# pedropro/UrsoNet

Measured on AMD Instinct MI355X. Metric: images/sec fwd+bwd ResNet50 640x512 bs32/GPU, higher is better.
Workload: dtype bf16; 1 GPU; resnet50 bottleneck=32 ori_resolution=16 soft-class head + loc regression, batch 32/GPU x 512x640x3, full training step (prep+fwd+loss+bwd+clip+SGD); global_batch=32, parallelism=dp1, comm_cus=0, hipgraph=True, runner=Engine, input=uint8 frames in HBM, mean subtraction + cast in the step (molding kernel), gradient_norm_from_finalisation_blocks=True, weight_gradients_on_forked_stream=True

## Files before the change

ursonet_amd/csrc/conv_c3.hip:

```cpp
#include "lds_mfma.h"
#include "internal.h"
#include <utility>

struct C3Args {
    const void* src; const void* wgt; const float* bias; const void* mask; void* dst;
    uint32_t bytes;
    int B, H, W, tiles_x, tiles_y, ntiles;
    int relu;
};

constexpr int C3_TH = 4, C3_TW = 32, C3_HW = C3_TW + 2, C3_HROWS = (C3_TH + 2) * C3_HW;
constexpr int C3_NA = 7;
constexpr int C3_ABUF = 224 * 128, C3_OOFF = 2 * C3_ABUF, C3_BOFF = C3_OOFF + C3_TH * C3_TW * 128, C3_LDS = C3_BOFF + 256;

__device__ __forceinline__ uint32_t c3_rd(int row, int h, int j) {
    const int s = (row >> 1) & 7;
    return (uint32_t)(row * 128 + ((((2 * j + h) ^ s)) << 4));
}

template <typename T, bool MASK>
__global__ __launch_bounds__(256, 2) void c3_kernel(const C3Args a) {
    static_assert(sizeof(T) == 2, "16-bit element types only");
    __shared__ __attribute__((aligned(1024))) char smem[C3_LDS];
    const uint32_t lds0 = (uint32_t)(uintptr_t)(__attribute__((address_space(3))) char*)smem;
    const int tid = threadIdx.x, lane = tid & 63, wave = __builtin_amdgcn_readfirstlane(tid >> 6);
    const int cw = wave & 1, pw = wave >> 1;
    int l31 = lane & 31;
    const int h = lane >> 5;

    const UrsoTileStream ts = urso_tile_stream(a.ntiles);
    const int t_end = ts.t_end, bpx = ts.bpx;
    int tile = ts.tile;
    if (tile >= t_end) return;

    const i32x4_t rs = raw_rsrc(a.src, a.bytes);
    const __amdgpu_buffer_rsrc_t rds = make_rsrc(a.dst, a.bytes);
    const __amdgpu_buffer_rsrc_t rmk = make_rsrc(MASK ? a.mask : a.dst, MASK ? a.bytes : 0u);

    int lane_d = lane;
    auto tile_origin = [&](int t, int& b, int& y0, int& x0) {
        const int tx = t % a.tiles_x, q = t / a.tiles_x;
        const int ty = q % a.tiles_y;
        b = q / a.tiles_y; y0 = ty * C3_TH; x0 = tx * C3_TW;
    };
    auto dma_tile = [&](int t, int buf) {
        int b, y0, x0;
        tile_origin(t, b, y0, x0);
        const int base = ((b * a.H + y0 - 1) * a.W + x0 - 1) * 128;
        asm volatile("" : "+v"(lane_d));
#pragma unroll
        for (int i = 0; i < C3_NA; ++i) {
            const int hr = 8 * (wave + 4 * i) + (lane_d >> 3);
            const int hy = (hr * 241) >> 13, hx = hr - hy * C3_HW;
            const int y = y0 - 1 + hy, x = x0 - 1 + hx;
            const bool ok = hr < C3_HROWS && y >= 0 && y < a.H && x >= 0 && x < a.W;
            const uint32_t off = (uint32_t)(base + (hy * a.W + hx) * 128 + (((lane_d & 7) ^ ((hx >> 1) & 7)) << 4));
            lds_dma16(rs, lds0 + buf * C3_ABUF + (wave + 4 * i) * 1024, ok ? off : URSO_OOB_SHIFT);
        }
    };

    i32x4_t wfr[9][4];
    {
        const int lg = 16 * ((l31 >> 2) & 1) + 4 * (l31 >> 3) + (l31 & 3);
        const char* wrow = (const char*)a.wgt + (size_t)(32 * cw + lg) * (9 * 64 * 2);
#pragma unroll
        for (int t = 0; t < 9; ++t)
#pragma unroll
            for (int j = 0; j < 4; ++j) wfr[t][j] = *(const i32x4_t*)(wrow + (t * 64 + 16 * j + 8 * h) * 2);
    }
    if (tid < 64) *(float*)(smem + C3_BOFF + tid * 4) = a.bias ? a.bias[tid] : 0.f;

    constexpr int NST = 4;
    uint32_t ea[3];
#pragma unroll
    for (int kx = 0; kx < 3; ++kx) ea[kx] = (uint32_t)(l31 * 128 + ((h ^ (((l31 + kx) >> 1) & 7)) << 4));

    dma_tile(tile, 0);
    int buf = 0;
    bool first = true;
    while (true) {
        const bool has_next = tile + bpx < t_end;
        if (first) wait_vm<0>(); else wait_vm<NST>();
        first = false;
        lds_barrier_asm();
        if (has_next) dma_tile(tile + bpx, buf ^ 1);

        f32x16_t acc[2];
        {
            const f32x4_t* bp = (const f32x4_t*)(smem + C3_BOFF + (32 * cw + 16 * h) * 4);
#pragma unroll
            for (int q = 0; q < 4; ++q) {
                const f32x4_t b4 = bp[q];
#pragma unroll
                for (int r = 0; r < 2; ++r) { acc[r][4 * q] = b4.x; acc[r][4 * q + 1] = b4.y; acc[r][4 * q + 2] = b4.z; acc[r][4 * q + 3] = b4.w; }
            }
        }
        i32x4_t f[4];
        uint32_t eb[3];
#pragma unroll
        for (int kx = 0; kx < 3; ++kx) eb[kx] = ea[kx] + (uint32_t)(buf * C3_ABUF + 2 * pw * C3_HW * 128);
        auto rd = [&](i32x4_t& fs, int s) {
            const int hr = s / 12, kx = (s / 4) % 3, j = s & 3;
            if (j == 0) asm volatile("" : "+v"(eb[kx]));
            fs = *(const i32x4_t*)(smem + (hr * C3_HW + kx) * 128 + (eb[kx] ^ (uint32_t)(j << 5)));
        };
        rd(f[0], 0);
        rd(f[1], 1);
        rd(f[2], 2);
#pragma unroll
        for (int s = 0; s < 48; ++s) {
            if (s + 3 < 48) rd(f[(s + 3) & 3], s + 3);
            __builtin_amdgcn_sched_barrier(0);
            const int hr = s / 12, kx = (s / 4) % 3, j = s & 3;
            if (hr <= 2) Mma32<T>::run(wfr[3 * hr + kx][j], f[s & 3], acc[0]);
            if (hr >= 1) Mma32<T>::run(wfr[3 * (hr - 1) + kx][j], f[s & 3], acc[1]);
            __builtin_amdgcn_sched_barrier(0);
        }

        char* sO = smem + C3_OOFF;
#pragma unroll
        for (int r = 0; r < 2; ++r) {
            const int px = (2 * pw + r) * 32 + l31;
#pragma unroll
            for (int v = 0; v < 2; ++v) {
                T o[8];
#pragma unroll
                for (int e = 0; e < 8; ++e) { float y = acc[r][8 * v + e]; y = a.relu ? relu_f(y) : y; o[e] = Elem<T>::from_f(y); }
                i32x4_t ov; __builtin_memcpy(&ov, o, 16);
                *(i32x4_t*)(sO + px * 128 + (((4 * cw + 2 * h + v) ^ ((px >> 1) & 7)) << 4)) = ov;
            }
        }
        int b, y0, x0;
        tile_origin(tile, b, y0, x0);
        uint32_t so[NST];
        i32x4_t mv[NST];
#pragma unroll
        for (int i = 0; i < NST; ++i) {
            const int row = 8 * (wave + 4 * i) + (lane >> 3);
            const int y = y0 + (row >> 5), x = x0 + (row & 31);
            so[i] = (y < a.H && x < a.W) ? (uint32_t)(((b * a.H + y) * a.W + x) * 128 + (((lane & 7) ^ ((row >> 1) & 7)) << 4)) : URSO_OOB_SHIFT;
            if constexpr (MASK) mv[i] = buf_load16(rmk, so[i]);
        }
        lds_barrier_asm();
#pragma unroll
        for (int i = 0; i < NST; ++i) {
            i32x4_t v = *(const i32x4_t*)(sO + (wave + 4 * i) * 1024 + lane * 16);
            if constexpr (MASK) {
                T x[8], m[8];
                __builtin_memcpy(x, &v, 16); __builtin_memcpy(m, &mv[i], 16);
#pragma unroll
                for (int e = 0; e < 8; ++e) x[e] = Elem<T>::to_f(m[e]) > 0.f ? x[e] : Elem<T>::from_f(0.f);
                __builtin_memcpy(&v, x, 16);
            }
            buf_store16(rds, so[i], v);
        }
        if (!has_next) break;
        tile += bpx; buf ^= 1;
    }
}

constexpr int C3W_PATCH = 2 * C3_ABUF;
constexpr int C3W_EOFF = 2 * C3W_PATCH, C3W_BOFF = C3W_EOFF + 8192, C3W_LDS = C3W_BOFF + 512;
constexpr int C3W_NA = 7;

template <typename T, bool MASK, int TW>
__global__ __launch_bounds__(512, 2) void c3w_kernel(const C3Args a) {
    constexpr int TH = 128 / TW, HW = TW + 2, HROWS = (TH + 2) * HW;
    static_assert(TW == 32 || TW == 16, "tile width");
    static_assert(sizeof(T) == 2, "16-bit element types only");
    __shared__ __attribute__((aligned(1024))) char smem[C3W_LDS];
    const uint32_t lds0 = (uint32_t)(uintptr_t)(__attribute__((address_space(3))) char*)smem;
    const int tid = threadIdx.x, lane = tid & 63, wave = __builtin_amdgcn_readfirstlane(tid >> 6);
    const int fq = wave & 3, ch = wave >> 2;
    int l31 = lane & 31;
    const int h = lane >> 5;

    const UrsoTileStream ts = urso_tile_stream(a.ntiles);
    const int t_end = ts.t_end, bpx = ts.bpx;
    int tile = ts.tile;
    if (tile >= t_end) return;

    const i32x4_t rs = raw_rsrc(a.src, a.bytes);
    const __amdgpu_buffer_rsrc_t rds = make_rsrc(a.dst, a.bytes);
    const __amdgpu_buffer_rsrc_t rmk = make_rsrc(MASK ? a.mask : a.dst, MASK ? a.bytes : 0u);

    int lane_d = lane;
    auto tile_origin = [&](int t, int& b, int& y0, int& x0) {
        const int tx = t % a.tiles_x, q = t / a.tiles_x;
        const int ty = q % a.tiles_y;
        b = q / a.tiles_y; y0 = ty * TH; x0 = tx * TW;
    };
    auto dma_tile = [&](int t, int buf) {
        int b, y0, x0;
        tile_origin(t, b, y0, x0);
        const int base = ((b * a.H + y0 - 1) * a.W + x0 - 1) * 256;
        asm volatile("" : "+v"(lane_d));
#pragma unroll
        for (int i = 0; i < C3W_NA; ++i) {
            const int ii = wave + 8 * i, half = ii >= 26 ? 1 : 0, rb = ii - 26 * half;
            const int hr = 8 * rb + (lane_d >> 3);
            const int hy = TW == 32 ? ((hr * 241) >> 13) : ((hr * 3641) >> 16), hx = hr - hy * HW;
            const int y = y0 - 1 + hy, x = x0 - 1 + hx;
            const bool ok = ii < 52 && hr < HROWS && y >= 0 && y < a.H && x >= 0 && x < a.W;
            const int sw = (hx >> 1) & 7;
            const uint32_t off = (uint32_t)(base + (hy * a.W + hx) * 256 + half * 128 + (((lane_d & 7) ^ sw) << 4));
            if (ii < 54) lds_dma16(rs, lds0 + buf * C3W_PATCH + half * C3_ABUF + rb * 1024, ok ? off : URSO_OOB_SHIFT);
        }
    };

    i32x4_t wfr[9][4];
    {
        const int lg = 16 * ((l31 >> 2) & 1) + 4 * (l31 >> 3) + (l31 & 3);
        const char* wrow = (const char*)a.wgt + (size_t)(32 * fq + lg) * (9 * 128 * 2);
#pragma unroll
        for (int t = 0; t < 9; ++t)
#pragma unroll
            for (int j = 0; j < 4; ++j) wfr[t][j] = *(const i32x4_t*)(wrow + (t * 128 + 64 * ch + 16 * j + 8 * h) * 2);
    }
    if (tid < 128) *(float*)(smem + C3W_BOFF + tid * 4) = a.bias ? a.bias[tid] : 0.f;

    constexpr int NST = 4;
    uint32_t ea[3];
    {
        const int prow = TW == 32 ? l31 : (l31 >> 4) * HW + (l31 & 15);
#pragma unroll
        for (int kx = 0; kx < 3; ++kx) ea[kx] = (uint32_t)(prow * 128 + ((h ^ ((((l31 & (TW - 1)) + kx) >> 1) & 7)) << 4));
    }
    dma_tile(tile, 0);
    int buf = 0;
    bool first = true;
    while (true) {
        const bool has_next = tile + bpx < t_end;
        if (first) wait_vm<0>(); else wait_vm<NST>();
        first = false;
        lds_barrier_asm();
        if (has_next) dma_tile(tile + bpx, buf ^ 1);
        f32x16_t acc[4];
#pragma unroll
        for (int r = 0; r < 4; ++r)
#pragma unroll
            for (int e = 0; e < 16; ++e) acc[r][e] = 0.f;
        i32x4_t f[4];
        uint32_t eb[3];
#pragma unroll
        for (int kx = 0; kx < 3; ++kx) eb[kx] = ea[kx] + (uint32_t)(buf * C3W_PATCH + ch * C3_ABUF);
        auto fresh = [&](int s) { if ((s & 3) == 0) asm volatile("" : "+v"(eb[(s / 4) % 3])); };
        if constexpr (TW == 32) {
            auto rd = [&](i32x4_t& fs, int s) {
                const int hr = s / 12, kx = (s / 4) % 3, j = s & 3;
                fresh(s);
                fs = *(const i32x4_t*)(smem + (hr * HW + kx) * 128 + (eb[kx] ^ (uint32_t)(j << 5)));
            };
            rd(f[0], 0);
            rd(f[1], 1);
            rd(f[2], 2);
#pragma unroll
            for (int s = 0; s < 72; ++s) {
                if (s + 3 < 72) rd(f[(s + 3) & 3], s + 3);
                __builtin_amdgcn_sched_barrier(0);
                const int hr = s / 12, kx = (s / 4) % 3, j = s & 3;
#pragma unroll
                for (int r = 0; r < 4; ++r) {
                    const int ky = hr - r;
                    if (ky >= 0 && ky <= 2) Mma32<T>::run(wfr[3 * ky + kx][j], f[s & 3], acc[r]);
                }
                __builtin_amdgcn_sched_barrier(0);
            }
        } else {
            auto rd = [&](i32x4_t& fs, int s) {
                const int rp = s / 12, kx = (s / 4) % 3, j = s & 3;
                fresh(s);
                fs = *(const i32x4_t*)(smem + (rp * HW + kx) * 128 + (eb[kx] ^ (uint32_t)(j << 5)));
            };
            rd(f[0], 0);
            rd(f[1], 1);
#pragma unroll
            for (int s = 0; s < 108; ++s) {
                if (s + 2 < 108) rd(f[(s + 2) % 3], s + 2);
                __builtin_amdgcn_sched_barrier(0);
                const int rp = s / 12, kx = (s / 4) % 3, j = s & 3;
#pragma unroll
                for (int m = 0; m < 4; ++m) {
                    const int ky = rp - 2 * m;
                    if (ky >= 0 && ky <= 2) Mma32<T>::run(wfr[3 * ky + kx][j], f[s % 3], acc[m]);
                }
                __builtin_amdgcn_sched_barrier(0);
            }
        }

        char* sX = smem + buf * C3W_PATCH;
        auto xoff = [&](int w, int rr, int q) -> char* {
            const uint32_t o = (uint32_t)(w * 8192 + ((rr * 4 + q) * 64 + lane) * 16);
            return (o < (uint32_t)C3W_PATCH) ? sX + o : smem + C3W_EOFF + (o - C3W_PATCH);
        };
        lds_barrier_asm();
#pragma unroll
        for (int rr = 0; rr < 2; ++rr) {
            const f32x16_t& v = (ch == 0) ? acc[2 + rr] : acc[rr];
#pragma unroll
            for (int q = 0; q < 4; ++q) *(f32x4_t*)xoff(wave, rr, q) = f32x4_t{v[4 * q], v[4 * q + 1], v[4 * q + 2], v[4 * q + 3]};
        }
        lds_barrier_asm();
        f32x16_t fin[2];
#pragma unroll
        for (int rr = 0; rr < 2; ++rr) {
            fin[rr] = (ch == 0) ? acc[rr] : acc[2 + rr];
#pragma unroll
            for (int q = 0; q < 4; ++q) {
                const f32x4_t p = *(const f32x4_t*)xoff(wave ^ 4, rr, q);
                fin[rr][4 * q] += p.x; fin[rr][4 * q + 1] += p.y; fin[rr][4 * q + 2] += p.z; fin[rr][4 * q + 3] += p.w;
            }
        }
        lds_barrier_asm();
        char* sO = sX;
        {
            const f32x4_t* bp = (const f32x4_t*)(smem + C3W_BOFF + (32 * fq + 16 * h) * 4);
#pragma unroll
            for (int rr = 0; rr < 2; ++rr) {
                const int px = (2 * ch + rr) * 32 + l31;
#pragma unroll
                for (int v = 0; v < 2; ++v) {
                    const f32x4_t b0 = bp[2 * v], b1 = bp[2 * v + 1];
                    const float bb[8] = {b0.x, b0.y, b0.z, b0.w, b1.x, b1.y, b1.z, b1.w};
                    T o[8];
#pragma unroll
                    for (int e = 0; e < 8; ++e) { float y = fin[rr][8 * v + e] + bb[e]; y = a.relu ? relu_f(y) : y; o[e] = Elem<T>::from_f(y); }
                    i32x4_t ov; __builtin_memcpy(&ov, o, 16);
                    *(i32x4_t*)(sO + px * 256 + (((4 * fq + 2 * h + v) ^ (px & 15)) << 4)) = ov;
                }
            }
        }
        int b, y0, x0;
        tile_origin(tile, b, y0, x0);
        uint32_t so[NST];
        i32x4_t mv[NST];
#pragma unroll
        for (int i = 0; i < NST; ++i) {
            const int p = (wave + 8 * i) * 64 + lane, px = p >> 4;
            const int y = y0 + px / TW, x = x0 + px % TW;
            so[i] = (y < a.H && x < a.W) ? (uint32_t)(((b * a.H + y) * a.W + x) * 256 + (((p & 15) ^ (px & 15)) << 4)) : URSO_OOB_SHIFT;
            if constexpr (MASK) mv[i] = buf_load16(rmk, so[i]);
        }
        lds_barrier_asm();
#pragma unroll
        for (int i = 0; i < NST; ++i) {
            i32x4_t v = *(const i32x4_t*)(sO + (wave + 8 * i) * 1024 + lane * 16);
            if constexpr (MASK) {
                T x[8], m[8];
                __builtin_memcpy(x, &v, 16); __builtin_memcpy(m, &mv[i], 16);
#pragma unroll
                for (int e = 0; e < 8; ++e) x[e] = Elem<T>::to_f(m[e]) > 0.f ? x[e] : Elem<T>::from_f(0.f);
                __builtin_memcpy(&v, x, 16);
            }
            buf_store16(rds, so[i], v);
        }
        if (!has_next) break;
        tile += bpx; buf ^= 1;
    }
}


#ifdef C3V_OLD_SWZ
__device__ __forceinline__ uint32_t c3v_swz(int col) { return (uint32_t)(col & 15); }
#else
__device__ __forceinline__ uint32_t c3v_swz(int col) { return (uint32_t)(0xfe64dcba98643210ull >> (4 * (col & 15))) & 15u; }
#endif
constexpr int C3V_HW = 18, C3V_HPIX = 10 * C3V_HW, C3V_PATCH = C3V_HPIX * 256;
constexpr int C3V_NA = 6;
#ifndef C3V_PF
#define C3V_PF 3
#endif
#ifndef C3V_DBG
#define C3V_DBG 0
#endif
#ifdef C3V_SEQ
__host__ __device__ constexpr int c3v_step(int t) { return t; }
#else
__host__ __device__ constexpr int c3v_step(int t) { return (t >> 1) + (t & 1) * 60; }
#endif
#ifdef C3V_NOSB
#define C3V_SB() do {} while (0)
#else
#define C3V_SB() __builtin_amdgcn_sched_barrier(0)
#endif
constexpr int C3V_OOFF = 2 * C3V_PATCH, C3V_BOFF = C3V_OOFF + 2 * 128 * 256, C3V_LDS = C3V_BOFF + 512;

template <class F, int... I> __device__ __forceinline__ void c3_static_for_impl(F&& f, std::integer_sequence<int, I...>) { (f(std::integral_constant<int, I>{}), ...); }
template <int N, class F> __device__ __forceinline__ void c3_static_for(F&& f) { c3_static_for_impl(static_cast<F&&>(f), std::make_integer_sequence<int, N>{}); }

template <typename T, bool MASK>
__global__ __launch_bounds__(512, 2) void c3v_kernel(const C3Args a) {
    static_assert(sizeof(T) == 2, "16-bit element types only");
    __shared__ __attribute__((aligned(1024))) char smem[C3V_LDS];
    const uint32_t lds0 = (uint32_t)(uintptr_t)(__attribute__((address_space(3))) char*)smem;
    const int tid = threadIdx.x, lane = tid & 63, wave = __builtin_amdgcn_readfirstlane(tid >> 6);
    const int fr = lane & 15, fg = lane >> 4;

    const UrsoTileStream ts = urso_tile_stream(a.ntiles);
    const int t_end = ts.t_end, bpx = ts.bpx;
    int tile = ts.tile;
    if (tile >= t_end) return;

    const i32x4_t rs = raw_rsrc(a.src, a.bytes);
    const __amdgpu_buffer_rsrc_t rds = make_rsrc(a.dst, a.bytes);
    const __amdgpu_buffer_rsrc_t rmk = make_rsrc(MASK ? a.mask : a.dst, MASK ? a.bytes : 0u);

    int lane_d = lane;
    auto tile_origin = [&](int t, int& b, int& y0, int& x0) {
        const int tx = t % a.tiles_x, q = t / a.tiles_x;
        const int ty = q % a.tiles_y;
        b = q / a.tiles_y; y0 = ty * 8; x0 = tx * 16;
    };
    auto dma_tile = [&](int t, int buf) {
        int b, y0, x0;
        tile_origin(t, b, y0, x0);
        const int base = ((b * a.H + y0 - 1) * a.W + x0 - 1) * 256;
        asm volatile("" : "+v"(lane_d));
#pragma unroll
        for (int i = 0; i < C3V_NA; ++i) {
            const int ii = wave + 8 * i;
            const int hp = 4 * ii + (lane_d >> 4);
            const int hy = (hp * 3641) >> 16, hx = hp - hy * C3V_HW;
            const int y = y0 - 1 + hy, x = x0 - 1 + hx;
            const bool ok = ii < 45 && y >= 0 && y < a.H && x >= 0 && x < a.W;
            const uint32_t off = (uint32_t)(base + (hy * a.W + hx) * 256 + (((uint32_t)(lane_d & 15) ^ c3v_swz(hx)) << 4));
            if (ii < 45) lds_dma16(rs, lds0 + buf * C3V_PATCH + ii * 1024, ok ? off : URSO_OOB_SHIFT);
        }
    };

    i32x4_t wfr[9][4];
    {
        const char* wrow = (const char*)a.wgt + (size_t)(16 * wave + fr) * (9 * 128 * 2);
#pragma unroll
        for (int t = 0; t < 9; ++t)
#pragma unroll
            for (int j = 0; j < 4; ++j) wfr[t][j] = *(const i32x4_t*)(wrow + (t * 128 + 32 * j + 8 * fg) * 2);
    }
    if (tid < 128) *(float*)(smem + C3V_BOFF + tid * 4) = a.bias ? a.bias[tid] : 0.f;

    uint32_t ea[3];
#pragma unroll
    for (int kx = 0; kx < 3; ++kx) ea[kx] = (uint32_t)((fr + kx) * 256) + (((uint32_t)fg ^ c3v_swz(fr + kx)) << 4);
    constexpr int NST = 4;
    uint32_t so[NST] = {URSO_OOB_SHIFT, URSO_OOB_SHIFT, URSO_OOB_SHIFT, URSO_OOB_SHIFT};
    i32x4_t mv[NST];
    auto flush = [&](int ob) {
        const char* sO = smem + C3V_OOFF + ob * (128 * 256);
#pragma unroll
        for (int i = 0; i < NST; ++i) {
            i32x4_t v = *(const i32x4_t*)(sO + (wave + 8 * i) * 1024 + lane * 16);
            if constexpr (MASK) {
                T x[8], m[8];
                __builtin_memcpy(x, &v, 16); __builtin_memcpy(m, &mv[i], 16);
#pragma unroll
                for (int e = 0; e < 8; ++e) x[e] = Elem<T>::to_f(m[e]) > 0.f ? x[e] : Elem<T>::from_f(0.f);
                __builtin_memcpy(&v, x, 16);
            }
            buf_store16(rds, so[i], v);
        }
    };
    dma_tile(tile, 0);
    int buf = 0, ob = 0;
    bool pend = false;
    while (true) {
        const bool has_next = tile + bpx < t_end;
        wait_vm<0>();
        lds_barrier_asm();
        if (has_next) dma_tile(tile + bpx, buf ^ 1);
        if (pend) flush(ob ^ 1);
        f32x4_t acc[8];
#pragma unroll
        for (int r = 0; r < 8; ++r) acc[r] = f32x4_t{0.f, 0.f, 0.f, 0.f};
        uint32_t eb[3];
#pragma unroll
        for (int kx = 0; kx < 3; ++kx) eb[kx] = ea[kx] + (uint32_t)(buf * C3V_PATCH);
        constexpr int PF = C3V_PF, RING = PF + 1;
        i32x4_t f[RING];
        auto rd = [&](i32x4_t& fs, int s) {
            const int hr = s / 12, kx = (s / 4) % 3, j = s & 3;
            if ((s & 3) == 0) asm volatile("" : "+v"(eb[kx]));
            if (!(C3V_DBG & 2) || s < PF) fs = *(const i32x4_t*)(smem + hr * C3V_HW * 256 + (eb[kx] ^ (uint32_t)(j << 6)));
        };
#pragma unroll
        for (int t = 0; t < PF; ++t) rd(f[t], c3v_step(t));
        c3_static_for<120>([&](auto sc) {
            constexpr int t = decltype(sc)::value, s = c3v_step(t);
            if constexpr (t + PF < 120) rd(f[(t + PF) % RING], c3v_step(t + PF));
            C3V_SB();
            constexpr int hr = s / 12, kx = (s / 4) % 3, j = s & 3;
            if (!(C3V_DBG & 1)) {
                if constexpr (hr >= 0 && hr < 8) Mma<T>::run(wfr[kx][j], f[t % RING], acc[hr]);
                if constexpr (hr - 1 >= 0 && hr - 1 < 8) Mma<T>::run(wfr[3 + kx][j], f[t % RING], acc[hr - 1]);
                if constexpr (hr - 2 >= 0 && hr - 2 < 8) Mma<T>::run(wfr[6 + kx][j], f[t % RING], acc[hr - 2]);
            }
            C3V_SB();
        });
        if (C3V_DBG & 4) { if (!has_next) break; tile += bpx; buf ^= 1; continue; }

        {
            char* sO = smem + C3V_OOFF + ob * (128 * 256);
            const f32x4_t bq = *(const f32x4_t*)(smem + C3V_BOFF + (16 * wave + 4 * fg) * 4);
#pragma unroll
            for (int r = 0; r < 8; ++r) {
                const int px = 16 * r + fr;
                float y0v = acc[r].x + bq.x, y1v = acc[r].y + bq.y, y2v = acc[r].z + bq.z, y3v = acc[r].w + bq.w;
                if (a.relu) { y0v = relu_f(y0v); y1v = relu_f(y1v); y2v = relu_f(y2v); y3v = relu_f(y3v); }
                T o[4] = {Elem<T>::from_f(y0v), Elem<T>::from_f(y1v), Elem<T>::from_f(y2v), Elem<T>::from_f(y3v)};
                i32x2_t ov; __builtin_memcpy(&ov, o, 8);
                *(i32x2_t*)(sO + px * 256 + ((((2 * wave + (fg >> 1)) ^ (px & 15))) << 4) + (fg & 1) * 8) = ov;
            }
        }
        {
            int b, y0, x0;
            tile_origin(tile, b, y0, x0);
#pragma unroll
            for (int i = 0; i < NST; ++i) {
                const int p = (wave + 8 * i) * 64 + lane, px = p >> 4;
                const int y = y0 + (px >> 4), x = x0 + (px & 15);
                so[i] = (y < a.H && x < a.W) ? (uint32_t)(((b * a.H + y) * a.W + x) * 256 + (((p & 15) ^ (px & 15)) << 4)) : URSO_OOB_SHIFT;
                if constexpr (MASK) mv[i] = buf_load16(rmk, so[i]);
            }
        }
        pend = true;
        if (!has_next) break;
        tile += bpx; buf ^= 1; ob ^= 1;
    }
    if constexpr (MASK) wait_vm<0>();
    lds_barrier_asm();
    flush(ob);
}

static int c3w_util(int H, int W, int tw) {
    const int th = 128 / tw;
    return (int)((long long)H * W * 100 / ((long long)ceil_div(H, th) * th * ceil_div(W, tw) * tw));
}
static int c3w_best_tw(int H, int W) { return c3w_util(H, W, 16) > c3w_util(H, W, 32) ? 16 : 32; }

bool urso_c3_fits(const urso_conv_geom* g, int dt, int flags, const void* add) {
    if (!g_urso_opt.c3 || add || (dt != URSO_BF16 && dt != URSO_F16) || (flags & (URSO_EPI_OUT_F32 | URSO_EPI_MASK_BITS | URSO_EPI_EMIT_BITS))) return false;
    if (g->KH != 3 || g->KW != 3 || g->SH != 1 || g->SW != 1 || g->PH != 1 || g->PW != 1 || g->DH != 1 || g->DW != 1 || g->FH > 0) return false;
    if (!((g->C == 64 && g->N == 64) || (g->C == 128 && g->N == 128 && (g_urso_opt.c3 == 1 || g_urso_opt.c3 == 3))) || g->OH != g->H || g->OW != g->W) return false;
    if (g->C == 128 && g_urso_opt.c3 == 1) {
        if (c3w_util(g->H, g->W, c3w_best_tw(g->H, g->W)) < 88) return false;
    }
    return (long long)g->B * g->H * g->W * g->C * 2 < 0x7FFFFF00ll;
}

int urso_c3_launch(const urso_conv_geom* g, int dt, int relu, const void* src, const void* wgt, const float* bias, const void* mask,
                   void* dst, hipStream_t st) {
    C3Args a;
    a.src = src; a.wgt = wgt; a.bias = bias; a.mask = mask; a.dst = dst; a.relu = relu;
    a.B = g->B; a.H = g->H; a.W = g->W;
    a.bytes = (uint32_t)((size_t)g->B * g->H * g->W * g->C * 2);
    const bool wide = g->C == 128;
    const int tw = wide ? c3w_best_tw(g->H, g->W) : C3_TW, th = 128 / tw;
    a.tiles_x = ceil_div(g->W, tw); a.tiles_y = ceil_div(g->H, th); a.ntiles = g->B * a.tiles_y * a.tiles_x;
    const dim3 grid(urso_persistent_grid(a.ntiles, wide ? 1 : 2)), blk(wide ? 512 : 256);
    if (wide) {
#define URSO_C3W(TT, TWV) do { if (mask) URSO_KLAUNCH((c3w_kernel<TT, true, TWV>), grid, blk, 0, st, a); \
                               else URSO_KLAUNCH((c3w_kernel<TT, false, TWV>), grid, blk, 0, st, a); } while (0)
        if (tw == 16 && g_urso_opt.c3v) {
            if (dt == URSO_BF16) { if (mask) URSO_KLAUNCH((c3v_kernel<__bf16, true>), grid, blk, 0, st, a); else URSO_KLAUNCH((c3v_kernel<__bf16, false>), grid, blk, 0, st, a); }
            else { if (mask) URSO_KLAUNCH((c3v_kernel<_Float16, true>), grid, blk, 0, st, a); else URSO_KLAUNCH((c3v_kernel<_Float16, false>), grid, blk, 0, st, a); }
            return urso_check_launch("urso_conv_igemm(3x3, 128 channels, 16-filter waves)");
        }
        if (dt == URSO_BF16) { if (tw == 32) URSO_C3W(__bf16, 32); else URSO_C3W(__bf16, 16); }
        else { if (tw == 32) URSO_C3W(_Float16, 32); else URSO_C3W(_Float16, 16); }
#undef URSO_C3W
        return urso_check_launch("urso_conv_igemm(3x3, 128 channels)");
    }
    if (dt == URSO_BF16) {
        if (mask) URSO_KLAUNCH((c3_kernel<__bf16, true>), grid, blk, 0, st, a);
        else URSO_KLAUNCH((c3_kernel<__bf16, false>), grid, blk, 0, st, a);
    } else {
        if (mask) URSO_KLAUNCH((c3_kernel<_Float16, true>), grid, blk, 0, st, a);
        else URSO_KLAUNCH((c3_kernel<_Float16, false>), grid, blk, 0, st, a);
    }
    return urso_check_launch("urso_conv_igemm(3x3, 64 channels)");
}
```

ursonet_amd/csrc/conv_c3g.hip:

```cpp
#include "lds_mfma.h"
#include "internal.h"

struct C3gArgs {
    const void* x; const void* dz; float* part; float* colpart; size_t part_stride;
    uint32_t bytes;
    int B, H, W, tiles_x, tiles_y, ntiles;
};

constexpr int CG_TH = 4, CG_TW = 32, CG_HW = CG_TW + 2, CG_HROWS = (CG_TH + 2) * CG_HW;
constexpr int CG_ABUF = 224 * 128, CG_ZOFF = CG_ABUF, CG_STAGE = CG_ABUF + CG_TH * CG_TW * 128, CG_LDS = 2 * CG_STAGE;

#ifndef CG_SWZ
#define CG_SWZ(r) ((((r) >> 1) & 1) << 2)
#endif

template <typename T, int TG>
__device__ __forceinline__ void cg_tile(const char* st, f32x16_t (&acc)[5], const uint32_t (&zoff)[2], const uint32_t (&abase)[8], bool csum) {
    const i32x4_t ones = {Elem<T>::ONES, Elem<T>::ONES, Elem<T>::ONES, Elem<T>::ONES};
#pragma unroll
    for (int ks = 0; ks < 8; ++ks) {
        const int ry = ks >> 1, hs = ks & 1;
        const uint32_t zb = (uint32_t)((32 * ry + 16 * hs) * 128);
        const i32x2_t zl = lds_read_tr16(st + zoff[0] + zb), zh = lds_read_tr16(st + zoff[1] + zb);
        const i32x4_t fz = i32x4_t{zl.x, zl.y, zh.x, zh.y};
#pragma unroll
        for (int i = 0; i < 5; ++i) {
            constexpr int dummy = 0; (void)dummy;
            const int tap = 5 * TG + i;
            if (tap == 9) { if (csum) Mma32<T>::run(ones, fz, acc[4]); continue; }
            const int ky = tap / 3, kx = tap - 3 * ky;
            constexpr int dummy2 = 0; (void)dummy2;
            const int c0 = (ry + ky) * CG_HW + 16 * hs + kx, c1 = c0 + 4;
            const i32x2_t al = lds_read_tr16(st + abase[c0 & 7] + c0 * 128);
            const i32x2_t ah = lds_read_tr16(st + abase[c1 & 7] + c1 * 128);
            Mma32<T>::run(i32x4_t{al.x, al.y, ah.x, ah.y}, fz, acc[i]);
        }
    }
}

template <typename T>
__global__ __launch_bounds__(512, 2) void c3g_kernel(const C3gArgs a) {
    static_assert(sizeof(T) == 2, "16-bit element types only");
    __shared__ __attribute__((aligned(1024))) char smem[CG_LDS];
    const uint32_t lds0 = (uint32_t)(uintptr_t)(__attribute__((address_space(3))) char*)smem;
    const int tid = threadIdx.x, lane = tid & 63, wave = __builtin_amdgcn_readfirstlane(tid >> 6);
    const int ct = wave & 1, nt = (wave >> 1) & 1, tg = wave >> 2;
    const int l31 = lane & 31, h = lane >> 5, l15 = lane & 15, g = lane >> 4;

    const UrsoTileStream ts = urso_tile_stream(a.ntiles);
    const int t_end = ts.t_end, bpx = ts.bpx;
    int tile = ts.tile;

    const i32x4_t rx = raw_rsrc(a.x, a.bytes), rz = raw_rsrc(a.dz, a.bytes);

    auto dma_tile = [&](int t, int buf) {
        const int tx = t % a.tiles_x, q = t / a.tiles_x, ty = q % a.tiles_y, b = q / a.tiles_y;
        const int y0 = ty * CG_TH, x0 = tx * CG_TW;
        const uint32_t sb = lds0 + buf * CG_STAGE;
#pragma unroll
        for (int i = 0; i < 4; ++i) {
            const int ii = wave + 8 * i;
            const int hr = 8 * ii + (lane >> 3);
            const int hy = (hr * 241) >> 13, hx = hr - hy * CG_HW;
            const int y = y0 - 1 + hy, x = x0 - 1 + hx;
            const bool ok = hr < CG_HROWS && y >= 0 && y < a.H && x >= 0 && x < a.W;
            const uint32_t off = (uint32_t)(((b * a.H + y) * a.W + x) * 128 + (((lane & 7) ^ CG_SWZ(hr)) << 4));
            if (ii < 26) lds_dma16(rx, sb + ii * 1024, ok ? off : URSO_OOB_SHIFT);
        }
#pragma unroll
        for (int i = 0; i < 2; ++i) {
            const int ii = wave + 8 * i;
            const int row = 8 * ii + (lane >> 3);
            const int y = y0 + (row >> 5), x = x0 + (row & 31);
            const bool ok = y < a.H && x < a.W;
            const uint32_t off = (uint32_t)(((b * a.H + y) * a.W + x) * 128 + (((lane & 7) ^ CG_SWZ(row)) << 4));
            lds_dma16(rz, sb + CG_ZOFF + ii * 1024, ok ? off : URSO_OOB_SHIFT);
        }
    };

    const int pix8 = 8 * (g >> 1) + (l15 >> 2);
    const int aslot = 2 * (2 * ct + (g & 1)) + ((l15 & 3) >> 1), abyte = ((l15 & 3) & 1) * 8;
    uint32_t abase[8];
#pragma unroll
    for (int j = 0; j < 8; ++j) abase[j] = (uint32_t)(pix8 * 128 + ((aslot ^ CG_SWZ(j + pix8)) << 4) + abyte);
    uint32_t zoff[2];
#pragma unroll
    for (int q = 0; q < 2; ++q) {
        const int row = pix8 + 4 * q;
        const int slot = 2 * (2 * nt + (g & 1)) + ((l15 & 3) >> 1);
        zoff[q] = (uint32_t)(CG_ZOFF + row * 128 + ((slot ^ CG_SWZ(row)) << 4) + ((l15 & 3) & 1) * 8);
    }

    f32x16_t acc[5];
#pragma unroll
    for (int i = 0; i < 5; ++i)
#pragma unroll
        for (int e = 0; e < 16; ++e) acc[i][e] = 0.f;
    const int tap0 = tg == 0 ? 0 : 5;
    const bool csum = tg == 1 && ct == 0;

    if (tile < t_end) dma_tile(tile, 0);
    int buf = 0;
    for (; tile < t_end; tile += bpx, buf ^= 1) {
        asm volatile("s_waitcnt vmcnt(0)" ::: "memory");
        __syncthreads();
        if (tile + bpx < t_end) dma_tile(tile + bpx, buf ^ 1);
        const char* st = smem + buf * CG_STAGE;
        if (tg == 0) cg_tile<T, 0>(st, acc, zoff, abase, false);
        else cg_tile<T, 1>(st, acc, zoff, abase, csum);
    }

    float* part = a.part + (size_t)blockIdx.x * a.part_stride;
#pragma unroll
    for (int i = 0; i < 5; ++i) {
        if (i == 4 && tg == 1) {
            if (csum && a.colpart && h == 0) a.colpart[(size_t)blockIdx.x * 64 + 32 * nt + l31] = acc[4][0];
            continue;
        }
        const int tap = tap0 + i;
#pragma unroll
        for (int r = 0; r < 16; ++r) part[(size_t)(64 * tap + 32 * ct + (r & 3) + 8 * (r >> 2) + 4 * h) * 64 + 32 * nt + l31] = acc[i][r];
    }
}

bool urso_c3g_fits(const urso_conv_geom* g, int dt) {
    if (!g_urso_opt.c3 || (dt != URSO_BF16 && dt != URSO_F16)) return false;
    if (g->KH != 3 || g->KW != 3 || g->SH != 1 || g->SW != 1 || g->PH != 1 || g->PW != 1 || g->DH != 1 || g->DW != 1 || g->FH > 0) return false;
    if (g->C != 64 || g->N != 64 || g->OH != g->H || g->OW != g->W) return false;
    return (long long)g->B * g->H * g->W * 128 < 0x7FFFFF00ll;
}
int urso_c3g_splits(const urso_conv_geom* g) {
    const int ntiles = g->B * ceil_div(g->H, CG_TH) * ceil_div(g->W, CG_TW);
    return urso_persistent_grid(ntiles, 1);
}
int urso_c3g_launch(const urso_conv_geom* g, int dt, const void* x, const void* dz, float* part, float* colpart, size_t part_stride, hipStream_t st) {
    C3gArgs a;
    a.x = x; a.dz = dz; a.part = part; a.colpart = colpart; a.part_stride = part_stride;
    a.B = g->B; a.H = g->H; a.W = g->W;
    a.bytes = (uint32_t)((size_t)g->B * g->H * g->W * 128);
    a.tiles_x = ceil_div(a.W, CG_TW); a.tiles_y = ceil_div(a.H, CG_TH); a.ntiles = a.B * a.tiles_y * a.tiles_x;
    const dim3 grid(urso_c3g_splits(g)), blk(512);
    if (dt == URSO_BF16) URSO_KLAUNCH((c3g_kernel<__bf16>), grid, blk, 0, st, a);
    else URSO_KLAUNCH((c3g_kernel<_Float16>), grid, blk, 0, st, a);
    return urso_check_launch("urso_conv_wgrad(c3)");
}
```

Measured before the change: 4698 images/sec.

## Triple-buffer c3 wgrad tiles and software-pipeline LDS reads with MFMAs

Converts the 3x3 64->64 weight-gradient kernel from a double-buffered loop with a full vmcnt(0) wait each tile to a three-stage LDS ring. Prefetch is issued two tiles ahead and the wait uses partial vmcnt counts. Inside a tile, LDS transpose reads for the next k-step are issued while the current MFMAs run, and scheduling group barriers interleave reads with MFMAs. The kernel is also split into compile-time tap-group/csum variants, and tile-invariant DMA address parts are precomputed. Debug macros that disable MMA or stores are added to both kernels but default to off. The deeper ring uses more LDS, which may limit blocks per CU, and adds register pressure from the double fragment buffers.

```diff
diff --git a/ursonet_amd/csrc/conv_c3.hip b/ursonet_amd/csrc/conv_c3.hip
--- a/ursonet_amd/csrc/conv_c3.hip
+++ b/ursonet_amd/csrc/conv_c3.hip
@@ -17,6 +17,10 @@
     const int s = (row >> 1) & 7;
     return (uint32_t)(row * 128 + ((((2 * j + h) ^ s)) << 4));
 }
+
+#ifndef C3_DBG
+#define C3_DBG 0
+#endif
 
 template <typename T, bool MASK>
 __global__ __launch_bounds__(256, 2) void c3_kernel(const C3Args a) {
@@ -83,7 +87,7 @@
         if (first) wait_vm<0>(); else wait_vm<NST>();
         first = false;
         lds_barrier_asm();
-        if (has_next) dma_tile(tile + bpx, buf ^ 1);
+        if (has_next && !(C3_DBG & 4)) dma_tile(tile + bpx, buf ^ 1);
 
         f32x16_t acc[2];
         {
@@ -112,9 +116,18 @@
             if (s + 3 < 48) rd(f[(s + 3) & 3], s + 3);
             __builtin_amdgcn_sched_barrier(0);
             const int hr = s / 12, kx = (s / 4) % 3, j = s & 3;
+            if constexpr (C3_DBG & 1) asm volatile("" :: "v"(f[s & 3]));
+            else {
             if (hr <= 2) Mma32<T>::run(wfr[3 * hr + kx][j], f[s & 3], acc[0]);
             if (hr >= 1) Mma32<T>::run(wfr[3 * (hr - 1) + kx][j], f[s & 3], acc[1]);
+            }
             __builtin_amdgcn_sched_barrier(0);
+        }
+        if constexpr (C3_DBG & 8) {
+            asm volatile("" :: "v"(acc[0]), "v"(acc[1]));
+            if (!has_next) break;
+            tile += bpx; buf ^= 1;
+            continue;
         }
 
         char* sO = smem + C3_OOFF;
@@ -152,7 +165,8 @@
                 for (int e = 0; e < 8; ++e) x[e] = Elem<T>::to_f(m[e]) > 0.f ? x[e] : Elem<T>::from_f(0.f);
                 __builtin_memcpy(&v, x, 16);
             }
-            buf_store16(rds, so[i], v);
+            if constexpr (C3_DBG & 2) asm volatile("" :: "v"(v));
+            else buf_store16(rds, so[i], v);
         }
         if (!has_next) break;
         tile += bpx; buf ^= 1;
diff --git a/ursonet_amd/csrc/conv_c3g.hip b/ursonet_amd/csrc/conv_c3g.hip
--- a/ursonet_amd/csrc/conv_c3g.hip
+++ b/ursonet_amd/csrc/conv_c3g.hip
@@ -8,33 +8,70 @@
 };
 
 constexpr int CG_TH = 4, CG_TW = 32, CG_HW = CG_TW + 2, CG_HROWS = (CG_TH + 2) * CG_HW;
-constexpr int CG_ABUF = 224 * 128, CG_ZOFF = CG_ABUF, CG_STAGE = CG_ABUF + CG_TH * CG_TW * 128, CG_LDS = 2 * CG_STAGE;
+constexpr int CG_ABUF = 224 * 128, CG_ZOFF = CG_ABUF, CG_STAGE = CG_ABUF + CG_TH * CG_TW * 128;
+constexpr int CG_NST = 3, CG_LDS = CG_NST * CG_STAGE;
+static_assert(CG_LDS <= 160 * 1024, "the ring has to fit the CU's LDS (one block per CU)");
 
 #ifndef CG_SWZ
 #define CG_SWZ(r) ((((r) >> 1) & 1) << 2)
 #endif
 
-template <typename T, int TG>
-__device__ __forceinline__ void cg_tile(const char* st, f32x16_t (&acc)[5], const uint32_t (&zoff)[2], const uint32_t (&abase)[8], bool csum) {
-    const i32x4_t ones = {Elem<T>::ONES, Elem<T>::ONES, Elem<T>::ONES, Elem<T>::ONES};
+#ifndef CG_DBG
+#define CG_DBG 0
+#endif
+
+template <int TG> struct CgFrag { i32x4_t z; i32x4_t a[5 - TG]; };
+
+template <int TG>
+__device__ __forceinline__ void cg_read(const char* st, int ks, CgFrag<TG>& f, const uint32_t (&zoff)[2], const uint32_t (&abase)[8]) {
+    const int ry = ks >> 1, hs = ks & 1;
+    const uint32_t zb = (uint32_t)((32 * ry + 16 * hs) * 128);
+    const i32x2_t zl = lds_read_tr16(st + zoff[0] + zb), zh = lds_read_tr16(st + zoff[1] + zb);
+    f.z = i32x4_t{zl.x, zl.y, zh.x, zh.y};
+#pragma unroll
+    for (int i = 0; i < 5 - TG; ++i) {
+        const int tap = 5 * TG + i, ky = tap / 3, kx = tap - 3 * ky;
+        const int c0 = (ry + ky) * CG_HW + 16 * hs + kx, c1 = c0 + 4;
+        const i32x2_t al = lds_read_tr16(st + abase[c0 & 7] + c0 * 128);
+        const i32x2_t ah = lds_read_tr16(st + abase[c1 & 7] + c1 * 128);
+        f.a[i] = i32x4_t{al.x, al.y, ah.x, ah.y};
+    }
+}
+template <typename T, int TG, bool CSUM>
+__device__ __forceinline__ void cg_mma(const CgFrag<TG>& f, f32x16_t (&acc)[5]) {
+    if constexpr (CG_DBG & 1) {
+#pragma unroll
+        for (int i = 0; i < 5 - TG; ++i) asm volatile("" :: "v"(f.a[i]), "v"(f.z));
+        return;
+    }
+#pragma unroll
+    for (int i = 0; i < 5 - TG; ++i) Mma32<T>::run(f.a[i], f.z, acc[i]);
+    if constexpr (TG == 1 && CSUM) {
+        const i32x4_t ones = {Elem<T>::ONES, Elem<T>::ONES, Elem<T>::ONES, Elem<T>::ONES};
+        Mma32<T>::run(ones, f.z, acc[4]);
+    }
+}
+template <int NR, int NM>
+__device__ __forceinline__ void cg_interleave() {
+    constexpr int G = NM - 1, Q = NR / G, R = NR % G;
+#pragma unroll
+    for (int m = 0; m < G; ++m) {
+        __builtin_amdgcn_sched_group_barrier(0x008, 1, 0);
+        if (m < R) __builtin_amdgcn_sched_group_barrier(0x100, Q + 1, 0);
+        else __builtin_amdgcn_sched_group_barrier(0x100, Q, 0);
+    }
+    __builtin_amdgcn_sched_group_barrier(0x008, 1, 0);
+}
+template <typename T, int TG, bool CSUM, typename Mid>
+__device__ __forceinline__ void cg_tile(const char* st, CgFrag<TG>& f0, CgFrag<TG>& f1, f32x16_t (&acc)[5], const uint32_t (&zoff)[2], const uint32_t (&abase)[8], Mid mid) {
+    constexpr int NR = 2 + 2 * (5 - TG), NM = 5 - TG + (TG == 1 && CSUM ? 1 : 0);
 #pragma unroll
     for (int ks = 0; ks < 8; ++ks) {
-        const int ry = ks >> 1, hs = ks & 1;
-        const uint32_t zb = (uint32_t)((32 * ry + 16 * hs) * 128);
-        const i32x2_t zl = lds_read_tr16(st + zoff[0] + zb), zh = lds_read_tr16(st + zoff[1] + zb);
-        const i32x4_t fz = i32x4_t{zl.x, zl.y, zh.x, zh.y};
-#pragma unroll
-        for (int i = 0; i < 5; ++i) {
-            constexpr int dummy = 0; (void)dummy;
-            const int tap = 5 * TG + i;
-            if (tap == 9) { if (csum) Mma32<T>::run(ones, fz, acc[4]); continue; }
-            const int ky = tap / 3, kx = tap - 3 * ky;
-            constexpr int dummy2 = 0; (void)dummy2;
-            const int c0 = (ry + ky) * CG_HW + 16 * hs + kx, c1 = c0 + 4;
-            const i32x2_t al = lds_read_tr16(st + abase[c0 & 7] + c0 * 128);
-            const i32x2_t ah = lds_read_tr16(st + abase[c1 & 7] + c1 * 128);
-            Mma32<T>::run(i32x4_t{al.x, al.y, ah.x, ah.y}, fz, acc[i]);
-        }
+        if (ks == 4) { mid(); __builtin_amdgcn_sched_barrier(0); }
+        if (ks < 7) cg_read<TG>(st, ks + 1, (ks & 1) ? f0 : f1, zoff, abase);
+        cg_mma<T, TG, CSUM>((ks & 1) ? f1 : f0, acc);
+        if (ks < 7) cg_interleave<NR, NM>();
+        __builtin_amdgcn_sched_barrier(0);
     }
 }
 
@@ -53,28 +90,32 @@
 
     const i32x4_t rx = raw_rsrc(a.x, a.bytes), rz = raw_rsrc(a.dz, a.bytes);
 
+    int py[6], px[6];
+    uint32_t prel[6];
+#pragma unroll
+    for (int i = 0; i < 4; ++i) {
+        const int hr = 8 * (wave + 8 * i) + (lane >> 3);
+        const int hy = (hr * 241) >> 13, hx = hr - hy * CG_HW;
+        py[i] = hr < CG_HROWS ? hy - 1 : -0x40000000; px[i] = hx - 1;
+        prel[i] = (uint32_t)(((hy - 1) * a.W + hx - 1) * 128 + (((lane & 7) ^ CG_SWZ(hr)) << 4));
+    }
+#pragma unroll
+    for (int i = 0; i < 2; ++i) {
+        const int row = 8 * (wave + 8 * i) + (lane >> 3);
+        py[4 + i] = row >> 5; px[4 + i] = row & 31;
+        prel[4 + i] = (uint32_t)(((row >> 5) * a.W + (row & 31)) * 128 + (((lane & 7) ^ CG_SWZ(row)) << 4));
+    }
     auto dma_tile = [&](int t, int buf) {
         const int tx = t % a.tiles_x, q = t / a.tiles_x, ty = q % a.tiles_y, b = q / a.tiles_y;
         const int y0 = ty * CG_TH, x0 = tx * CG_TW;
-        const uint32_t sb = lds0 + buf * CG_STAGE;
-#pragma unroll
-        for (int i = 0; i < 4; ++i) {
-            const int ii = wave + 8 * i;
-            const int hr = 8 * ii + (lane >> 3);
-            const int hy = (hr * 241) >> 13, hx = hr - hy * CG_HW;
-            const int y = y0 - 1 + hy, x = x0 - 1 + hx;
-            const bool ok = hr < CG_HROWS && y >= 0 && y < a.H && x >= 0 && x < a.W;
-            const uint32_t off = (uint32_t)(((b * a.H + y) * a.W + x) * 128 + (((lane & 7) ^ CG_SWZ(hr)) << 4));
-            if (ii < 26) lds_dma16(rx, sb + ii * 1024, ok ? off : URSO_OOB_SHIFT);
-        }
-#pragma unroll
-        for (int i = 0; i < 2; ++i) {
-            const int ii = wave + 8 * i;
-            const int row = 8 * ii + (lane >> 3);
-            const int y = y0 + (row >> 5), x = x0 + (row & 31);
-            const bool ok = y < a.H && x < a.W;
-            const uint32_t off = (uint32_t)(((b * a.H + y) * a.W + x) * 128 + (((lane & 7) ^ CG_SWZ(row)) << 4));
-            lds_dma16(rz, sb + CG_ZOFF + ii * 1024, ok ? off : URSO_OOB_SHIFT);
+        const uint32_t sb = lds0 + buf * CG_STAGE, t0 = (uint32_t)(((b * a.H + y0) * a.W + x0) * 128);
+#pragma unroll
+        for (int i = 0; i < 6; ++i) {
+            const int ii = wave + 8 * (i < 4 ? i : i - 4);
+            const bool ok = (uint32_t)(y0 + py[i]) < (uint32_t)a.H && (uint32_t)(x0 + px[i]) < (uint32_t)a.W;
+            const uint32_t off = ok ? t0 + prel[i] : URSO_OOB_SHIFT;
+            if (i >= 4) lds_dma16(rz, sb + CG_ZOFF + ii * 1024, off);
+            else if (ii < 26) lds_dma16(rx, sb + ii * 1024, off);
         }
     };
 
@@ -99,16 +140,30 @@
     const int tap0 = tg == 0 ? 0 : 5;
     const bool csum = tg == 1 && ct == 0;
 
-    if (tile < t_end) dma_tile(tile, 0);
-    int buf = 0;
-    for (; tile < t_end; tile += bpx, buf ^= 1) {
-        asm volatile("s_waitcnt vmcnt(0)" ::: "memory");
-        __syncthreads();
-        if (tile + bpx < t_end) dma_tile(tile + bpx, buf ^ 1);
-        const char* st = smem + buf * CG_STAGE;
-        if (tg == 0) cg_tile<T, 0>(st, acc, zoff, abase, false);
-        else cg_tile<T, 1>(st, acc, zoff, abase, csum);
-    }
+    auto walk = [&](auto tgc, auto csc) {
+        constexpr int TG = decltype(tgc)::value;
+        constexpr bool CSUM = decltype(csc)::value;
+        CgFrag<TG> f0, f1;
+        if (tile < t_end) dma_tile(tile, 0);
+        if (tile + bpx < t_end) dma_tile(tile + bpx, 1);
+        int stage = 0;
+        for (; tile < t_end; tile += bpx) {
+            if (tile + bpx >= t_end) wait_vm<0>();
+            else if (wave < 2) wait_vm<6>();
+            else wait_vm<5>();
+            lds_barrier_asm();
+            const char* st = smem + stage * CG_STAGE;
+            cg_read<TG>(st, 0, f0, zoff, abase);
+            auto request = [&]() { if (!(CG_DBG & 4) && tile + 2 * bpx < t_end) dma_tile(tile + 2 * bpx, stage == 0 ? 2 : stage - 1); };
+            if constexpr (TG == 0) request();
+            __builtin_amdgcn_sched_barrier(0);
+            cg_tile<T, TG, CSUM>(st, f0, f1, acc, zoff, abase, [&]() { if constexpr (TG == 1) request(); });
+            stage = stage == 2 ? 0 : stage + 1;
+        }
+    };
+    if (tg == 0) walk(std::integral_constant<int, 0>{}, std::false_type{});
+    else if (csum) walk(std::integral_constant<int, 1>{}, std::true_type{});
+    else walk(std::integral_constant<int, 1>{}, std::false_type{});
 
     float* part = a.part + (size_t)blockIdx.x * a.part_stride;
 #pragma unroll
```

Result: no change. 4710 images/sec, median of 6 (+0.3%).
